# alpapad/java-rsync

Hardware: AMD Instinct MI355X
Metric: GiB/s device-resident rolling+MD5 scan (Generator block sums + Sender match scan; bytes read) (higher is better)
Workload: dtype u8

## Files before the change

### include/rsync_hip_debug.h

```cpp
#ifndef RSYNC_HIP_DEBUG_H
#define RSYNC_HIP_DEBUG_H

#include <stdint.h>

#include "rsync_hip.h"

#ifdef __cplusplus
extern "C" {
#endif

int rsh_debug_set_option(const char* name, int64_t value);
int rsh_debug_get_option(const char* name, int64_t* value);
void rsh_debug_reset_options(void);

int rsh_debug_kernel_ms(rsh_ctx* ctx, int32_t which, double* ms);

int rsh_debug_generation(rsh_ctx* ctx, int32_t set, int32_t* gen);

int rsh_debug_streams_busy(rsh_ctx* ctx, int32_t* mask);

int rsh_debug_k1_clock(rsh_ctx* ctx, const void* d_data, int64_t n, int32_t block_length, int32_t reps,
                       double* clock_ghz);

int rsh_debug_multi_selftest(const int64_t* bytes, int32_t njobs, int32_t nparts, int32_t fail_part, int32_t* part_out,
                             int32_t* order_out, int32_t* status_out);

int rsh_debug_tokens_selftest(const uint8_t* src, int64_t n, const rsh_event* ev, int64_t n_ev,
                              const uint8_t file_md5[16], int64_t from, uint8_t* out, int64_t len, int64_t span,
                              int64_t* n_desc);

int rsh_debug_sums_selftest(int32_t unframe, const rsh_header* h, int32_t* weak, uint8_t* strong, uint8_t* wire,
                            int64_t len, int64_t span, int64_t* n_desc);

typedef struct {
    int64_t pos;
    int32_t kind;
    int32_t value;
// ... 13 lines not shown
```

### java-rsync_amd/csrc/capi.cpp

```cpp
#include <hip/hip_runtime.h>
#include <immintrin.h>
#include <stdio.h>
#include <stdlib.h>
#include <string.h>

#include <algorithm>
#include <atomic>
#include <chrono>
#include <functional>
#include <thread>
#include <vector>

#include "device.h"
#include "host_md5.h"
#include "resolver.h"
#include "rsync_hip.h"

#include "ctx.h"
#include "options.h"
#include "rsync_hip_debug.h"

namespace {
int warm_calls(rsh_ctx* c) {
    const uint8_t seed[4] = {1, 2, 3, 4};
// ... 477 lines not shown
    rsh::opt_table()[i].store(value, std::memory_order_relaxed);
    return RSH_OK;
}

int rsh_debug_get_option(const char* name, int64_t* value) {
    const int i = rsh::opt_index(name);
    if (i < 0 || !value) return RSH_E_INVAL;
    *value = rsh::opt((rsh::Opt)i);
    return RSH_OK;
}

void rsh_debug_reset_options(void) {
    for (int i = 0; i < rsh::OPT_COUNT; ++i) rsh::opt_table()[i].store(rsh::opt_info()[i].def, std::memory_order_relaxed);
}

int rsh_debug_kernel_ms(rsh_ctx* ctx, int32_t which, double* ms) {
    if (!ctx || !ms || which < 0 || which > 2) return RSH_E_INVAL;
    *ms = -1.0;
    const bool timed = which == 0 ? ctx->gen_timed : which == 1 ? ctx->spec_timed : ctx->sums_timed;
    if (!timed) return RSH_OK;
    const hipEvent_t a = which == 0 ? ctx->ev_gen_a : which == 1 ? ctx->ev_k1a : ctx->ev_sums_a;
    const hipEvent_t b = which == 0 ? ctx->ev_gen_b : which == 1 ? ctx->ev_k1b : ctx->ev_sums_b;
    RSH_HIP(hipSetDevice(ctx->device));
    RSH_HIP(hipEventSynchronize(b));
    float f = 0.f;
    RSH_HIP(hipEventElapsedTime(&f, a, b));
    *ms = f;
    return RSH_OK;
}

// ... 55 lines not shown
```

### java-rsync_amd/csrc/device.h

```cpp
#pragma once
#include <hip/hip_runtime.h>
#include <stdint.h>

#include <vector>

#include "hit_cache.h"
#include "rsync_hip.h"

namespace rsh {

hipError_t launch_block_sums(const uint8_t* d_data, int64_t n, uint32_t B, uint32_t nchunks, uint32_t dl,
                             uint32_t seed_word, int32_t* d_weak, uint8_t* d_strong, hipStream_t s,
                             const int* abort_flag = nullptr, int abort_gen = 0);
void k1_timing_next(hipEvent_t start, hipEvent_t stop);
bool k1_timing_taken();

#ifdef RSH_KBENCH
hipError_t launch_block_sums_variant(int variant, const uint8_t* d_data, int64_t n, uint32_t B, uint32_t nchunks,
                                     uint32_t dl, uint32_t seed_word, int32_t* d_weak, uint8_t* d_strong,
                                     hipStream_t s, const int* abort_flag = nullptr, int abort_gen = 0);
#endif

struct K1File {
    const uint8_t* data;
// ... 41 lines not shown
struct K1Plan {
    const uint8_t* data;
    int32_t* weak;
    uint8_t* strong;
    uint32_t B, dl;
    uint32_t g0, ng;
    const int* abort = nullptr;
    int32_t file = 0;
    uint32_t nfull = 0;
};
uint32_t plan_block_sums_files(const K1File* files, int32_t nfiles, std::vector<K1Plan>* plans,
                               std::vector<K1Lane>* lanes, int* lane_align, bool* partial = nullptr);
hipError_t launch_expand_groups(const K1Plan* d_plans, uint32_t nplans, uint32_t ngroups, K1Group* d_groups,
                                hipStream_t s);
bool tail_gather_on();
hipError_t launch_block_sums_batch(const K1Group* d_groups, uint32_t ngroups, const K1Lane* d_lanes, uint32_t nlanes,
                                   int lane_align, uint32_t seed_word, hipStream_t s, const int* abort_flag = nullptr,
                                   int abort_gen = 0, bool partial = false);

hipError_t launch_chain_flags(const int32_t* d_wsrc, const uint8_t* d_ssrc, const int32_t* d_wbas,
                              const uint8_t* d_sbas, uint32_t count, uint32_t dl, uint8_t* d_flags,
                              hipStream_t s);
hipError_t launch_warm_k1(hipStream_t s);
hipError_t launch_warm_scan(hipStream_t s);
hipError_t launch_warm_chain(hipStream_t s);
hipError_t launch_warm_io(hipStream_t s);
constexpr uint32_t kStampGroups = 64, kStampLine = 16;
struct Stamp {
    uint32_t* counter;
    int* stamp;
// ... 258 lines not shown
```

### java-rsync_amd/csrc/device.hip

```cpp
#include <hip/hip_ext.h>
#include <hip/hip_runtime.h>

#include "device.h"
#include "device_common.h"
#include "md5_core.h"
#include "options.h"

#include <algorithm>
#include <type_traits>

namespace rsh {

__device__ __forceinline__ void weak_block(const uint32_t (&m)[16], int32_t& s1, int32_t& u, uint32_t off) {
    int32_t a = 0, b = 0;
#pragma unroll
    for (int j = 0; j < 16; ++j) {
        a = __builtin_amdgcn_sdot4((int)m[j], 0x01010101, a, false);
        const int w = (4 * j) | ((4 * j + 1) << 8) | ((4 * j + 2) << 16) | ((4 * j + 3) << 24);
        b = __builtin_amdgcn_sdot4((int)m[j], w, b, false);
    }
    s1 += a;
    u += (int32_t)(off * (uint32_t)a) + b;
}

// ... 193 lines not shown
    return v;
}

__device__ __forceinline__ void compiler_fence() { asm volatile("" ::: "memory"); }

__device__ __forceinline__ void md5_stream_block(Md5State& st, const uint32_t (&m)[16]) { md5_compress_rot16n(st, m); }

#ifndef RSH_K1_TAIL_PF
#define RSH_K1_TAIL_PF 2
#endif
#ifdef RSH_K1_NUMVGPR
#define K1_PIPE_ATTR __attribute__((amdgpu_num_vgpr(RSH_K1_NUMVGPR)))
#else
#define K1_PIPE_ATTR __attribute__((amdgpu_waves_per_eu(3)))
#endif
template <bool MULTI = false, bool GATHER = false, bool WEAKV = false>
__device__ __forceinline__ void block_sums_pipe_body(const uint8_t* __restrict__ data, uint32_t B, uint32_t dl,
                                                             uint32_t seed, int32_t* __restrict__ weak_out,
                                                             uint8_t* __restrict__ strong_out,
                                                             const int* abort_flag = nullptr, int abort_gen = 0,
                                                             const K1Group* __restrict__ groups = nullptr,
                                                             int64_t n = 0, uint32_t nchunks = 0,
                                                             uint32_t main_waves = 0xFFFFFFFFu,
                                                             const K1Tail* __restrict__ gt = nullptr,
                                                             uint32_t gcnt = 0, uint32_t gsel = 0xFFFFFFFFu) {
    constexpr int ROW = 9;
    constexpr int BUF = 64 * ROW;
    constexpr int TAIL_PF = RSH_K1_TAIL_PF;
    if constexpr (!MULTI && !GATHER) {
        if (blockIdx.x >= main_waves) {
            const uint32_t c = main_waves * 64u + (blockIdx.x - main_waves) * 64u + threadIdx.x;
// ... 40 lines not shown
    {
        const int m = l & 15, q = l >> 4, type = m >> 2;
#pragma unroll
        for (int w = 0; w < 4; ++w)
#pragma unroll
            for (int d = 0; d < 4; ++d) {
                uint32_t word = 0;
                if (q == (m & 3) && type == 0) word = 0x01010101u;
                else if (q == (m & 3) && type == 1)
#pragma unroll
                    for (int b = 0; b < 4; ++b) word |= (uint32_t)(16 * w + 4 * d + b) << (8 * b);
                wW[w][d] = (int)word;
            }
    }

    uint4 q[2][8];
    uint4 Wa[4];
    uint4 Wb[4];
    const __amdgpu_buffer_rsrc_t rsrc =
        __builtin_amdgcn_make_buffer_rsrc(const_cast<uint8_t*>(gdata), 0, (int)(64 * B), 0x00020000);
    const uint32_t lane_off = (uint32_t)(l >> 3) * B + 16u * (uint32_t)(l & 7);
    auto load = [&](uint4 (&dst)[8], uint32_t stg) __attribute__((always_inline)) {
#pragma unroll
        for (int j = 0; j < 8; ++j) {
            if constexpr (GATHER) {
                dst[j] = ld16<false>(rp[j] + 128u * stg);
            } else {
                const u32x4 t = __builtin_amdgcn_raw_buffer_load_b128(rsrc, lane_off + 128u * stg, (int)(j * 8u * B), 2);
                dst[j] = make_uint4(t.x, t.y, t.z, t.w);
            }
        }
    };
    auto put = [&](const uint4 (&src)[8], int buf) __attribute__((always_inline)) {
#pragma unroll
        for (int j = 0; j < 8; ++j) lds_all[buf * BUF + wr0 + j * 8 * ROW] = src[j];
    };
    auto get_words = [&](uint4 (&w)[4], int buf, int h) __attribute__((always_inline)) {
#pragma unroll
        for (int k = 0; k < 4; ++k) w[k] = lds_all[buf * BUF + rd0 + 4 * h + k];
    };
    Md5State st = md5_init();
    auto md5_block = [&](const uint4 (&w)[4]) __attribute__((always_inline)) {
        uint32_t m[16];
        unpack(w, m);
        md5_stream_block(st, m);
    };
    [[maybe_unused]] int32_t vs1 = 0, vu = 0;
    auto weak_words = [&](const uint4 (&w)[4], [[maybe_unused]] uint32_t off) __attribute__((always_inline)) {
        if constexpr (WEAKV) {
            uint32_t m[16];
            unpack(w, m);
            weak_block(m, vs1, vu, off);
        } else {
#pragma unroll
            for (int e = 0; e < 4; ++e) RW[e] += accW[e];
#pragma unroll
            for (int k = 0; k < 4; ++k) {
                const v4i32 b4 = {(int)w[k].x, (int)w[k].y, (int)w[k].z, (int)w[k].w};
                accW = __builtin_amdgcn_mfma_i32_16x16x64_i8(wW[k], b4, accW, 0, 0, 0);
            }
        }
    };
    auto stage = [&](auto pc, uint32_t si, bool has_next, bool refill) __attribute__((always_inline)) {
        constexpr int P = decltype(pc)::value;
        if (has_next) {
            put(q[P ^ 1], P ^ 1);
            if (refill) load(q[P ^ 1], si + 3);
        }
        get_words(Wb, P, 1);
        md5_block(Wa);
        weak_words(Wa, 128u * si);
        compiler_fence();
        if (has_next) get_words(Wa, P ^ 1, 0);
        md5_block(Wb);
        weak_words(Wb, 128u * si + 64u);
        compiler_fence();
// ... 11 lines not shown
    compiler_fence();
    get_words(Wa, 0, 0);
    uint32_t s = 0;
    int flag = 0;
    for (; s + 5 <= nst && flag != abort_gen; s += 2) {
        asm volatile("s_load_dword %0, %1, 0x0 glc" : "=s"(flag) : "s"(abort_flag));
        stage(std::integral_constant<int, 0>{}, s, true, true);
        stage(std::integral_constant<int, 1>{}, s + 1, true, true);
        asm volatile("s_waitcnt lgkmcnt(0)" : "+s"(flag));
    }
    if (flag == abort_gen) return;
    for (; s < nst; s += 2) {
        stage(std::integral_constant<int, 0>{}, s, s + 1 < nst, s + 3 < nst);
        if (s + 1 < nst) stage(std::integral_constant<int, 1>{}, s + 1, s + 2 < nst, s + 4 < nst);
    }
    {
        const uint64_t bits = ((uint64_t)B + 4) * 8;
        uint32_t m[16] = {seed, 0x80u, 0, 0, 0, 0, 0, 0, 0, 0, 0, 0, 0, 0, (uint32_t)bits, (uint32_t)(bits >> 32)};
        md5_compress(st, m);
    }
    int32_t s1, u;
    if constexpr (WEAKV) {
        s1 = vs1;
        u = vu;
    } else {
#pragma unroll
        for (int e = 0; e < 4; ++e) RW[e] += accW[e];
        const int n = l & 15, q = l >> 4;
        int32_t tS[4], tR[4], tW[4];
#pragma unroll
// ... 11 lines not shown
    uint32_t c = c0 + l;
    if constexpr (GATHER) {
        if ((uint32_t)l >= gcnt) return;
        if (gt) {
            const K1Tail t = gt[l];
            weak_out = t.weak;
            strong_out = t.strong;
            c = t.c;
        }
    }
    const int32_t s2 = (int32_t)(B * (uint32_t)s1 - (uint32_t)u);
    weak_out[c] = (int32_t)(((uint32_t)s1 & 0xFFFFu) | ((uint32_t)s2 << 16));
    store_digest(strong_out + (size_t)c * dl, st, dl);
}

template <bool MULTI = false>
__global__ __launch_bounds__(64) K1_PIPE_ATTR void block_sums_pipe_kernel(const uint8_t* __restrict__ data, uint32_t B, uint32_t dl,
                                                             uint32_t seed, int32_t* __restrict__ weak_out,
                                                             uint8_t* __restrict__ strong_out,
                                                             const int* abort_flag = nullptr, int abort_gen = 0,
                                                             const K1Group* __restrict__ groups = nullptr,
                                                             int64_t n = 0, uint32_t nchunks = 0,
                                                             uint32_t main_waves = 0xFFFFFFFFu) {
    block_sums_pipe_body<MULTI>(data, B, dl, seed, weak_out, strong_out, abort_flag, abort_gen, groups, n, nchunks,
                                main_waves);
}
__global__ __launch_bounds__(64) __attribute__((amdgpu_num_vgpr(256))) void block_sums_pipe_tailg_kernel(
    const uint8_t* __restrict__ data, uint32_t B, uint32_t dl, uint32_t seed, int32_t* __restrict__ weak_out,
    uint8_t* __restrict__ strong_out, const int* abort_flag, int abort_gen, int64_t n, uint32_t nchunks,
    uint32_t main_waves, uint32_t tail_full) {
    if (blockIdx.x >= main_waves) {
        const uint32_t tw = blockIdx.x - main_waves, ngw = (tail_full + 63u) / 64u;
        if (tw < ngw) {
            const uint32_t first = main_waves * 64u + 64u * tw;
            block_sums_pipe_body<false, true>(
                data + (size_t)first * B, B, dl, seed, weak_out + first, strong_out + (size_t)first * dl, abort_flag,
                abort_gen, nullptr, 0, 0, 0xFFFFFFFFu, nullptr, min(64u, tail_full - 64u * tw));
            return;
        }
        const uint32_t c = main_waves * 64u + tail_full + (tw - ngw) * 64u + threadIdx.x;
        if (c < nchunks) lane_chunk_sums<16, RSH_K1_TAIL_PF, false>(data, n, B, c, dl, seed, weak_out, strong_out);
        return;
    }
    block_sums_pipe_body<false>(data, B, dl, seed, weak_out, strong_out, abort_flag, abort_gen, nullptr, n, nchunks,
                                main_waves);
}
bool tail_gather_on() { return opt(OPT_K1_GATHER) != 0; }
#ifdef RSH_KBENCH
__global__ __launch_bounds__(64) K1_PIPE_ATTR void block_sums_pipe_weakv_kernel(
    const uint8_t* __restrict__ data, uint32_t B, uint32_t dl, uint32_t seed, int32_t* __restrict__ weak_out,
    uint8_t* __restrict__ strong_out, const int* abort_flag, int abort_gen) {
    block_sums_pipe_body<false, false, true>(data, B, dl, seed, weak_out, strong_out, abort_flag, abort_gen);
}
#endif

__global__ __launch_bounds__(64) K1_PIPE_ATTR void block_sums_pipe_clock_kernel(
    const uint8_t* __restrict__ data, uint32_t B, uint32_t dl, uint32_t seed, int32_t* __restrict__ weak_out,
    uint8_t* __restrict__ strong_out, const int* abort_flag, int abort_gen, int64_t n, uint32_t nchunks,
    unsigned long long* __restrict__ clk) {
    const uint64_t c0 = __builtin_amdgcn_s_memtime(), r0 = __builtin_amdgcn_s_memrealtime();
    block_sums_pipe_body<false>(data, B, dl, seed, weak_out, strong_out, abort_flag, abort_gen, nullptr, n, nchunks,
                                0xFFFFFFFFu);
    const uint64_t c1 = __builtin_amdgcn_s_memtime(), r1 = __builtin_amdgcn_s_memrealtime();
    if (threadIdx.x == 0) {
        atomicAdd(&clk[0], (unsigned long long)(c1 - c0));
        atomicAdd(&clk[1], (unsigned long long)(r1 - r0));
    }
}

hipError_t launch_k1_clock(const uint8_t* d_data, int64_t n, uint32_t B, uint32_t dl, uint32_t seed_word,
                           int32_t* d_weak, uint8_t* d_strong, unsigned long long* d_clk, hipStream_t s) {
    if (B == 0 || B % 128 != 0 || n <= 0 || n % (64 * (int64_t)B) != 0 || dl > 16) return hipErrorInvalidValue;
    const uint32_t nchunks = (uint32_t)(n / B), waves = nchunks / 64;
    const size_t wave_lds = 64 * 9 * sizeof(uint4);
    hipLaunchKernelGGL(block_sums_pipe_clock_kernel, dim3(waves), dim3(64), 2 * wave_lds, s, d_data, B, dl, seed_word,
                       d_weak, d_strong, never_word(), -1, n, nchunks, d_clk);
    return hipGetLastError();
}
#ifndef RSH_K1_SHIFT_VGPR
#define RSH_K1_SHIFT_VGPR 256
#endif
template <int W>
__device__ __forceinline__ void shift_wave(const uint8_t* __restrict__ gdata, uint32_t a, uint32_t B, uint32_t dl,
                                           uint32_t seed, int32_t* __restrict__ weak_out,
                                           uint8_t* __restrict__ strong_out, const int* abort_flag, int abort_gen) {
    constexpr int ROW = 17;
    extern __shared__ __attribute__((aligned(16))) uint4 lds_all[];
    const int l = threadIdx.x;
    const uint32_t nst = B >> 7;
    const uint32_t Q = a >> 4, r = a & 3;
    const int wr0 = (l >> 3) * ROW + (l & 7);
// ... 203 lines not shown
        t_k1_taken = true;
    } else {
        hipLaunchKernelGGL(kernel, grid, block, lds, s, static_cast<KArgs>(args)...);
    }
}

#ifndef RSH_KBENCH
static
#endif
hipError_t launch_block_sums_variant(int variant, const uint8_t* d_data, int64_t n, uint32_t B, uint32_t nchunks,
                                     uint32_t dl, uint32_t seed_word, int32_t* d_weak, uint8_t* d_strong,
                                     hipStream_t s, const int* abort_flag, int abort_gen) {
    if (nchunks == 0) return hipSuccess;
    const uintptr_t addr = reinterpret_cast<uintptr_t>(d_data);
    const uint32_t nst = B >> 7;
#ifdef RSH_KBENCH
    if (variant == 1010) {
        if ((B % 128) != 0 || nst < 4 || nst > 1024 || n != (int64_t)nchunks * B || nchunks % 64 != 0 || (addr % 128) != 0)
            return hipErrorInvalidValue;
        hipLaunchKernelGGL(block_sums_pipe_weakv_kernel, dim3(nchunks / 64), dim3(64), 2 * 64 * 9 * sizeof(uint4), s,
                           d_data, B, dl, seed_word, d_weak, d_strong, abort_flag ? abort_flag : never_word(),
                           abort_flag ? abort_gen : -1);
        return hipGetLastError();
    }
#endif
    const bool coalesced = variant < 0 && abort_flag && (B % 128) == 0 && nst >= 4 && nst <= 1024;
    if (coalesced && (addr % 128) != 0 && opt(OPT_K1_SHIFT) != 0) {
        hipDeviceptr_t lo = nullptr;
        size_t size = 0;
        const uint32_t a = (uint32_t)(addr % 128);
        if (hipMemGetAddressRange(&lo, &size, reinterpret_cast<hipDeviceptr_t>(const_cast<uint8_t*>(d_data))) ==
// ... 29 lines not shown
                    default:
                        k1_launch(block_sums_shift_kernel<3>, grid, dim3(64), (uint32_t)lb, s, d_data, n, a, B, nchunks,
                                  mw, dl, seed_word, d_weak, d_strong, abort_flag, abort_gen, tf);
                }
                return hipGetLastError();
            }
        }
    }
    const uint32_t waves = (uint32_t)std::min<int64_t>(n / B, nchunks) / 64;
    if (coalesced && waves > 0 && ((addr % 16) == 0 || opt(OPT_K1_UNALIGNED) != 0)) {
        const uint32_t nfullc = (uint32_t)std::min<int64_t>(n / B, nchunks);
        const size_t wave_lds = 64 * 9 * sizeof(uint4);
        const uint32_t tail_waves = (nchunks - 64 * waves + 63) / 64;
        const uint32_t tail_full = nfullc - 64 * waves, tail_short = nchunks - nfullc;
        const uint32_t gwaves = (tail_full + 63) / 64 + (tail_short + 63) / 64;
        if (tail_full > 0 && tail_gather_on() && (gwaves == tail_waves || waves + gwaves <= 2 * 4 * kCUs)) {
            k1_launch(block_sums_pipe_tailg_kernel, dim3(waves + gwaves), dim3(64), (uint32_t)(2 * wave_lds), s, d_data,
                      B, dl, seed_word, d_weak, d_strong, abort_flag, abort_gen, n, nchunks, waves, tail_full);
            return hipGetLastError();
        }
        k1_launch(block_sums_pipe_kernel<false>, dim3(waves + tail_waves), dim3(64), (uint32_t)(2 * wave_lds), s,
                  d_data, B, dl, seed_word, d_weak, d_strong, abort_flag, abort_gen, nullptr, n, nchunks, waves);
        return hipGetLastError();
    }
    const dim3 block(64);
    const dim3 grid((nchunks + 63) / 64);
    if ((B % 16) == 0 && (addr % 16) == 0) {
        hipLaunchKernelGGL((block_sums_kernel<16, 4, true>), grid, block, 0, s, d_data, n, B, nchunks, dl, seed_word,
                           d_weak, d_strong, 0u);
    } else if ((B % 4) == 0 && (addr % 4) == 0) {
        hipLaunchKernelGGL((block_sums_kernel<4, 2>), grid, block, 0, s, d_data, n, B, nchunks, dl, seed_word, d_weak,
                           d_strong, 0u);
    } else {
        hipLaunchKernelGGL((block_sums_kernel<0, 4, false>), grid, block, 0, s, d_data, n, B, nchunks, dl, seed_word,
                           d_weak, d_strong, 0u);
    }
    return hipGetLastError();
// ... 102 lines not shown
}

static const int* never_word() {
    static int* ptr[64] = {};
    int dev = 0;
    if (hipGetDevice(&dev) != hipSuccess || dev < 0 || dev >= 64) return nullptr;
    if (!ptr[dev]) {
        int* p = nullptr;
        if (hipExtMallocWithFlags(reinterpret_cast<void**>(&p), 256, hipDeviceMallocUncached) != hipSuccess) return nullptr;
        if (hipMemset(p, 0, 256) != hipSuccess) return nullptr;
        ptr[dev] = p;
    }
    return ptr[dev];
}

template <int ALIGN>
__global__ __launch_bounds__(64) __attribute__((amdgpu_num_vgpr(256))) void block_sums_pipe_multi_g_kernel(
    const K1Group* __restrict__ groups, uint32_t ngroups, const K1Lane* __restrict__ lanes, uint32_t seed,
    const int* abort_flag, int abort_gen) {
    if (blockIdx.x >= ngroups) {
        const K1Lane e = lanes[blockIdx.x - ngroups];
        const uint32_t c = e.c_first + threadIdx.x;
        if (c < e.nchunks)
            lane_chunk_sums<ALIGN == 1 ? 0 : ALIGN, ALIGN == 16 ? 4 : ALIGN == 4 ? 2 : 4, ALIGN != 1>(
                e.data, e.n, e.B, c, e.dl, seed, e.weak, e.strong);
        return;
    }
    const K1Group g = groups[blockIdx.x];
    if (g.count < 64) {
        block_sums_pipe_body<false, true>(g.data, g.B, g.dl, seed, g.weak, g.strong,
                                                           g.abort ? g.abort : abort_flag, abort_gen, nullptr, 0, 0,
                                                           0xFFFFFFFFu, nullptr, g.count);
        return;
    }
    block_sums_pipe_body<true>(nullptr, 0u, 0u, seed, nullptr, nullptr, abort_flag, abort_gen, groups);
}

hipError_t launch_block_sums_batch(const K1Group* d_groups, uint32_t ngroups, const K1Lane* d_lanes, uint32_t nlanes,
                                   int lane_align, uint32_t seed_word, hipStream_t s, const int* abort_flag,
                                   int abort_gen, bool partial) {
    const size_t lb = 2 * 64 * 9 * sizeof(uint4);
    if (!abort_flag && (abort_flag = never_word()) != nullptr) abort_gen = -1;
    if (!abort_flag) return hipErrorOutOfMemory;
    if (partial || (tail_gather_on() && nlanes > 0 && ngroups > 0)) {
        const dim3 grid(ngroups + nlanes);
        if (lane_align == 16)
            hipLaunchKernelGGL((block_sums_pipe_multi_g_kernel<16>), grid, dim3(64), lb, s, d_groups, ngroups, d_lanes,
                               seed_word, abort_flag, abort_gen);
        else if (lane_align == 4)
            hipLaunchKernelGGL((block_sums_pipe_multi_g_kernel<4>), grid, dim3(64), lb, s, d_groups, ngroups, d_lanes,
                               seed_word, abort_flag, abort_gen);
        else
            hipLaunchKernelGGL((block_sums_pipe_multi_g_kernel<1>), grid, dim3(64), lb, s, d_groups, ngroups, d_lanes,
                               seed_word, abort_flag, abort_gen);
        return hipGetLastError();
    }
    if (ngroups > 0)
        hipLaunchKernelGGL((block_sums_pipe_kernel<true>), dim3(ngroups), dim3(64), lb, s, nullptr, 0u, 0u, seed_word,
                           nullptr, nullptr, abort_flag, abort_gen, d_groups);
    if (nlanes > 0) {
        if (lane_align == 16)
            hipLaunchKernelGGL((block_sums_lane_batch_kernel<16>), dim3(nlanes), dim3(64), 0, s, d_lanes, seed_word);
        else if (lane_align == 4)
            hipLaunchKernelGGL((block_sums_lane_batch_kernel<4>), dim3(nlanes), dim3(64), 0, s, d_lanes, seed_word);
        else
            hipLaunchKernelGGL((block_sums_lane_batch_kernel<1>), dim3(nlanes), dim3(64), 0, s, d_lanes, seed_word);
    }
    return hipGetLastError();
}

hipError_t launch_block_sums(const uint8_t* d_data, int64_t n, uint32_t B, uint32_t nchunks, uint32_t dl,
                             uint32_t seed_word, int32_t* d_weak, uint8_t* d_strong, hipStream_t s,
                             const int* abort_flag, int abort_gen) {
    if (!abort_flag && (abort_flag = never_word()) != nullptr) abort_gen = -1;
// ... 32 lines not shown
```

### java-rsync_amd/csrc/options.h

```cpp
#pragma once
#include <stdint.h>
#include <string.h>

#include <atomic>

namespace rsh {

enum Opt : int {
    OPT_K1_GATHER,
    OPT_K1_SHIFT,
    OPT_K1_UNALIGNED,
    OPT_SCAN_TRACE,
    OPT_SCAN_SEGMENTED,
    OPT_SCAN_SAMPLES,
    OPT_BATCH_CHAIN,
    OPT_BATCH_CHAIN_PREFIX,
    OPT_HOST_CORES,
    OPT_FILE_TILE,
    OPT_FILE_TILE_ABOVE,
    OPT_PROBE_LONG,
    OPT_SEGMENT_BYTES,
    OPT_MD5_WIDTH,
    OPT_CHAIN_HELPERS,
    OPT_CHAIN_MAP_BYTES,
    OPT_TIME_GEN,
    OPT_BATCH_WARM,
    OPT_FAULT_INJECT,
    OPT_TOKENS_SPAN,
    OPT_TOKENS_PIECE,
    OPT_SUMS_PIECE,
    OPT_TOKENS_RUNS,
    OPT_COUNT
};

struct OptInfo {
    const char* name;
    int64_t def;
};

inline constexpr OptInfo kOpts[OPT_COUNT] = {
    {"k1_gather", 1},           {"k1_shift", 1},        {"k1_unaligned", 1},
    {"scan_trace", 0},          {"scan_segmented", 1},  {"scan_samples", 256},
    {"batch_chain", 1},         {"batch_chain_prefix", -1}, {"host_cores", 0},
    {"file_tile", 4LL << 30},   {"file_tile_above", 32LL << 30}, {"probe_long", 1},
    {"segment_bytes", 16LL << 30}, {"md5_width", 0},    {"chain_helpers", -1},
    {"chain_map_bytes", 1LL << 30}, {"time_gen", 1},    {"batch_warm", 128},
    {"fault_inject", 0},        {"tokens_span", 256LL << 10}, {"tokens_piece", 8LL << 20},
    {"sums_piece", 32LL << 20}, {"tokens_runs", 64LL << 10},
};

inline const OptInfo* opt_info() { return kOpts; }

inline std::atomic<int64_t>* opt_table() {
    static std::atomic<int64_t> v[OPT_COUNT] = {};
    static std::atomic<bool> init{false};
    if (!init.load(std::memory_order_acquire)) {
        static std::atomic_flag once = ATOMIC_FLAG_INIT;
        if (!once.test_and_set()) {
            for (int i = 0; i < OPT_COUNT; ++i) v[i].store(kOpts[i].def, std::memory_order_relaxed);
            init.store(true, std::memory_order_release);
        } else {
            while (!init.load(std::memory_order_acquire)) {
            }
// ... 15 lines not shown
```

### java-rsync_amd/rsync_hip.py

```python
import ctypes
import os
import subprocess

import numpy as np

HERE = os.path.dirname(os.path.abspath(__file__))
LIB_PATH = os.environ.get("RSH_LIB") or os.path.join(HERE, "lib", "librsynchip.so")

RSH_OK, RSH_E_INVAL, RSH_E_PROTOCOL, RSH_E_OVERFLOW, RSH_E_NOSPACE, RSH_E_DEVICE, RSH_E_NOMEM, RSH_E_BUSY = \
    0, -1, -2, -3, -4, -5, -6, -7
RSH_E_NOTFOUND, RSH_E_OPEN, RSH_E_NOSOURCE = -8, -9, -10
EV_LITERAL, EV_MATCH = 1, 2


class ProtocolError(Exception):
    """RsyncProtocolException (Connection.receiveChecksumHeader, Connection.java:28-38)."""


class FileViewNotFound(FileNotFoundError):
    """RSH_E_NOTFOUND (io/FileViewNotFound: new FileView on a missing file, FileView.java:74-75)."""


class FileViewOpenFailed(OSError):
    """RSH_E_OPEN (io/FileViewOpenFailed, FileView.java:76-78)."""
# ... 120 lines not shown
                        ("count", "<i4"), ("reserved", "<i4")])

EXPORTS = ["rsh_abi_version", "rsh_strerror", "rsh_last_error", "rsh_device_count", "rsh_ctx_create", "rsh_ctx_destroy",
           "rsh_ctx_stream", "rsh_block_length_for", "rsh_digest_length_for", "rsh_header_make",
           "rsh_header_validate", "rsh_block_sums", "rsh_block_sums_device", "rsh_ctx_sync", "rsh_ctx_trim", "rsh_match_scan",
           "rsh_match_scan_device", "rsh_match_scan_tiled", "rsh_fetch_events", "rsh_file_md5", "rsh_tokens_size", "rsh_tokens_write", "rsh_generator_bytes",
           "rsh_block_sums_batch_device", "rsh_match_scan_batch_device", "rsh_receiver_combine",
           "rsh_receiver_combine_device", "rsh_receiver_combine_batch", "rsh_block_sums_file", "rsh_match_scan_file", "rsh_block_sums_pieces", "rsh_match_scan_pieces", "rsh_block_sums_batch", "rsh_match_scan_batch", "rsh_block_sums_batch_multi", "rsh_match_scan_batch_multi", "rsh_receiver_combine_batch_multi", "rsh_shard_files", "rsh_file_md5_batch", "rsh_dev_alloc", "rsh_dev_free", "rsh_memcpy_h2d", "rsh_memcpy_d2h", "rsh_fill_splitmix_device",
           "rsh_tokens_write_device", "rsh_tokens_write_kept", "rsh_tokens_write_batch_device",
           "rsh_sums_wire_size", "rsh_header_from_wire", "rsh_sums_frame_device", "rsh_sums_unframe_device",
           "rsh_block_sums_batch_wire", "rsh_match_scan_batch_wire", "rsh_block_sums_batch_wire_multi",
           "rsh_match_scan_batch_wire_multi", "rsh_tokens_frame_device", "rsh_receiver_combine_resident"]
DEBUG_EXPORTS = ["rsh_debug_set_option", "rsh_debug_get_option", "rsh_debug_reset_options", "rsh_debug_k1_clock",
                 "rsh_debug_streams_busy", "rsh_debug_kernel_ms", "rsh_debug_multi_selftest", "rsh_debug_generation",
                 "rsh_debug_tokens_selftest", "rsh_debug_sums_selftest", "rsh_debug_tokens_scan_selftest",
                 "rsh_debug_untokens_selftest"]

_LIB = None


def build(force=False):
    cmd = ["make", "-s", "-C", HERE] + (["-B"] if force else [])
    subprocess.run(cmd, check=True)


def stale_sources():
    import hashlib
    stamp = os.path.splitext(LIB_PATH)[0] + ".srchash"
    if not os.path.exists(stamp):
        return []
    out = []
# ... 62 lines not shown
        "rsh_match_scan_batch": ([P, ctypes.POINTER(ScanBatchJob), I32, P, ctypes.POINTER(ScanStats)], ctypes.c_int),
        "rsh_block_sums_batch_multi": ([ctypes.POINTER(P), I32, ctypes.POINTER(BlockBatchJob), I32, P], ctypes.c_int),
        "rsh_match_scan_batch_multi": ([ctypes.POINTER(P), I32, ctypes.POINTER(ScanBatchJob), I32, P,
                                        ctypes.POINTER(ScanStats)], ctypes.c_int),
        "rsh_receiver_combine_batch_multi": ([ctypes.POINTER(P), I32, ctypes.POINTER(CombineJob), I32], ctypes.c_int),
        "rsh_shard_files": ([P, I32, I32, P], ctypes.c_int),
        "rsh_file_md5_batch": ([ctypes.POINTER(Md5Job), I32, I32], ctypes.c_int),
        "rsh_dev_alloc": ([P, I64, ctypes.POINTER(P)], ctypes.c_int),
        "rsh_dev_free": ([P, P], ctypes.c_int),
        "rsh_memcpy_h2d": ([P, P, P, I64], ctypes.c_int),
        "rsh_memcpy_d2h": ([P, P, P, I64], ctypes.c_int),
        "rsh_fill_splitmix_device": ([P, P, I64, ctypes.c_uint64, I64], ctypes.c_int),
        "rsh_debug_set_option": ([ctypes.c_char_p, I64], ctypes.c_int),
        "rsh_debug_get_option": ([ctypes.c_char_p, ctypes.POINTER(I64)], ctypes.c_int),
        "rsh_debug_reset_options": ([], None),
        "rsh_debug_k1_clock": ([P, P, I64, I32, I32, ctypes.POINTER(ctypes.c_double)], ctypes.c_int),
        "rsh_debug_streams_busy": ([P, ctypes.POINTER(ctypes.c_int32)], ctypes.c_int),
        "rsh_debug_generation": ([P, I32, ctypes.POINTER(ctypes.c_int32)], ctypes.c_int),
        "rsh_debug_kernel_ms": ([P, I32, ctypes.POINTER(ctypes.c_double)], ctypes.c_int),
        "rsh_debug_multi_selftest": ([P, I32, I32, I32, P, P, P], ctypes.c_int),
        "rsh_tokens_write_device": ([P, P, I64, P, I64, P, I64, P, I64], ctypes.c_int),
        "rsh_tokens_write_kept": ([P, P, I64, P, I64, P, I64], ctypes.c_int),
        "rsh_tokens_write_batch_device": ([P, ctypes.POINTER(TokenJob), I32], ctypes.c_int),
        "rsh_debug_tokens_selftest": ([P, I64, P, I64, P, I64, P, I64, I64, ctypes.POINTER(I64)], ctypes.c_int),
        "rsh_sums_wire_size": ([HP], I64),
        "rsh_header_from_wire": ([P, HP], ctypes.c_int),
        "rsh_sums_frame_device": ([P, HP, P, P, P, I64], ctypes.c_int),
        "rsh_sums_unframe_device": ([P, HP, P, I64, P, P], ctypes.c_int),
        "rsh_block_sums_batch_wire": ([P, ctypes.POINTER(BlockWireJob), I32, P], ctypes.c_int),
        "rsh_match_scan_batch_wire": ([P, ctypes.POINTER(SendJob), I32, P, ctypes.POINTER(ScanStats)], ctypes.c_int),
# ... 714 lines not shown
```

Baseline: 5142.

## Stream K1 block-sum input via buffer_load-to-LDS DMA with swizzled staging

Adds a DMA path to the block-sums pipeline kernel. Raw buffer_load ... lds instructions copy each 128-byte stage straight into LDS using an XOR-swizzled layout, instead of routing the data through VGPRs and then writing it to LDS. Reads are double-buffered with vmcnt-based waits and abort polling through scalar loads. The goal is to cut VGPR traffic and instruction overhead in the memory-bound MD5/weak-sum loop. The cost is hand-written inline asm that manipulates m0, a fixed 16 KiB LDS footprint, and a new option, enabled by default, that falls back to the old register path.

```diff
diff --git a/include/rsync_hip_debug.h b/include/rsync_hip_debug.h
--- a/include/rsync_hip_debug.h
+++ b/include/rsync_hip_debug.h
@@ -21,6 +21,8 @@
 
 int rsh_debug_k1_clock(rsh_ctx* ctx, const void* d_data, int64_t n, int32_t block_length, int32_t reps,
                        double* clock_ghz);
+
+int32_t rsh_debug_k1_dma_swizzle(int32_t what, int32_t chunk, int32_t index);
 
 int rsh_debug_multi_selftest(const int64_t* bytes, int32_t njobs, int32_t nparts, int32_t fail_part, int32_t* part_out,
                              int32_t* order_out, int32_t* status_out);
diff --git a/java-rsync_amd/csrc/capi.cpp b/java-rsync_amd/csrc/capi.cpp
--- a/java-rsync_amd/csrc/capi.cpp
+++ b/java-rsync_amd/csrc/capi.cpp
@@ -515,6 +515,12 @@
     for (int i = 0; i < rsh::OPT_COUNT; ++i) rsh::opt_table()[i].store(rsh::opt_info()[i].def, std::memory_order_relaxed);
 }
 
+int32_t rsh_debug_k1_dma_swizzle(int32_t what, int32_t chunk, int32_t index) {
+    if (what < 0 || what > 2 || chunk < 0 || chunk > 63 || index < 0 || index > 7) return -1;
+    const uint32_t c = (uint32_t)chunk, i = (uint32_t)index;
+    return (int32_t)(what == 0 ? rsh::k1_dma_piece(c, i) : what == 1 ? rsh::k1_dma_slot(c, i) : rsh::k1_dma_lds_byte(c, i));
+}
+
 int rsh_debug_kernel_ms(rsh_ctx* ctx, int32_t which, double* ms) {
     if (!ctx || !ms || which < 0 || which > 2) return RSH_E_INVAL;
     *ms = -1.0;
diff --git a/java-rsync_amd/csrc/device.h b/java-rsync_amd/csrc/device.h
--- a/java-rsync_amd/csrc/device.h
+++ b/java-rsync_amd/csrc/device.h
@@ -79,6 +79,11 @@
 hipError_t launch_expand_groups(const K1Plan* d_plans, uint32_t nplans, uint32_t ngroups, K1Group* d_groups,
                                 hipStream_t s);
 bool tail_gather_on();
+constexpr uint32_t K1_DMA_STAGE = 8192;
+constexpr uint32_t k1_dma_piece(uint32_t c, uint32_t p) { return p ^ ((c >> 1) & 7u); }
+constexpr uint32_t k1_dma_slot(uint32_t c, uint32_t k) { return k ^ ((c >> 1) & 7u); }
+constexpr uint32_t k1_dma_lds_byte(uint32_t c, uint32_t slot) { return 128u * c + 16u * slot; }
+bool k1_dma_on();
 hipError_t launch_block_sums_batch(const K1Group* d_groups, uint32_t ngroups, const K1Lane* d_lanes, uint32_t nlanes,
                                    int lane_align, uint32_t seed_word, hipStream_t s, const int* abort_flag = nullptr,
                                    int abort_gen = 0, bool partial = false);
diff --git a/java-rsync_amd/csrc/device.hip b/java-rsync_amd/csrc/device.hip
--- a/java-rsync_amd/csrc/device.hip
+++ b/java-rsync_amd/csrc/device.hip
@@ -231,7 +231,7 @@
 #else
 #define K1_PIPE_ATTR __attribute__((amdgpu_waves_per_eu(3)))
 #endif
-template <bool MULTI = false, bool GATHER = false, bool WEAKV = false>
+template <bool MULTI = false, bool GATHER = false, bool WEAKV = false, bool DMA = false, int DIAG = 0>
 __device__ __forceinline__ void block_sums_pipe_body(const uint8_t* __restrict__ data, uint32_t B, uint32_t dl,
                                                              uint32_t seed, int32_t* __restrict__ weak_out,
                                                              uint8_t* __restrict__ strong_out,
@@ -302,8 +302,140 @@
             }
     }
 
+    Md5State st = md5_init();
+    auto md5_block = [&](const uint4 (&w)[4]) __attribute__((always_inline)) {
+        if constexpr (DIAG == 2) {
+#pragma unroll
+            for (int k = 0; k < 4; ++k) st.a ^= w[k].x ^ w[k].y ^ w[k].z ^ w[k].w;
+            return;
+        }
+        uint32_t m[16];
+        unpack(w, m);
+        md5_stream_block(st, m);
+    };
+    [[maybe_unused]] int32_t vs1 = 0, vu = 0;
+    auto weak_words = [&](const uint4 (&w)[4], [[maybe_unused]] uint32_t off) __attribute__((always_inline)) {
+        if constexpr (DIAG == 2) return;
+        if constexpr (WEAKV) {
+            uint32_t m[16];
+            unpack(w, m);
+            weak_block(m, vs1, vu, off);
+        } else {
+#pragma unroll
+            for (int e = 0; e < 4; ++e) RW[e] += accW[e];
+#pragma unroll
+            for (int k = 0; k < 4; ++k) {
+                const v4i32 b4 = {(int)w[k].x, (int)w[k].y, (int)w[k].z, (int)w[k].w};
+                accW = __builtin_amdgcn_mfma_i32_16x16x64_i8(wW[k], b4, accW, 0, 0, 0);
+            }
+        }
+    };
+    uint4 Wa[4];
+    if constexpr (DMA) {
+        static_assert(!GATHER && !WEAKV, "the DMA form is the main waves' form only");
+        B = (uint32_t)__builtin_amdgcn_readfirstlane((int)B);
+        const uint64_t ga = reinterpret_cast<uint64_t>(gdata);
+        const v4i32 desc = {__builtin_amdgcn_readfirstlane((int)(uint32_t)ga),
+                            __builtin_amdgcn_readfirstlane((int)((uint32_t)(ga >> 32) & 0xFFFFu)),
+                            DIAG == 1 ? 0 : (int)(64u * B),
+                            0x00020000};
+        const uint32_t lds0 = __builtin_amdgcn_readfirstlane(
+            (int)(uint32_t)reinterpret_cast<uintptr_t>((__attribute__((address_space(3))) void*)lds_all));
+        const uint32_t voff = (uint32_t)(l >> 3) * B + 16u * k1_dma_piece((uint32_t)(l >> 3), (uint32_t)(l & 7));
+        const uint32_t so1 = 8u * B, so2 = 16u * B, so3 = 24u * B, so4 = 32u * B, so5 = 40u * B, so6 = 48u * B,
+                       so7 = 56u * B;
+        auto dma = [&](int slot, uint32_t stg) __attribute__((always_inline)) {
+            uint32_t keep;
+            const uint32_t ve = voff + 128u * stg, vo = ve ^ 64u;
+            asm volatile(
+                "s_nop 4\n\t"
+                "s_waitcnt lgkmcnt(0)\n\t"
+                "s_mov_b32 %0, m0\n\t"
+                "s_mov_b32 m0, %4\n\t"
+                "s_nop 0\n\t"
+                "buffer_load_dwordx4 %2, %1, 0 offen nt lds\n\t"
+                "s_add_u32 m0, m0, 0x400\n\t"
+                "s_nop 0\n\t"
+                "buffer_load_dwordx4 %3, %1, %5 offen nt lds\n\t"
+                "s_add_u32 m0, m0, 0x400\n\t"
+                "s_nop 0\n\t"
+                "buffer_load_dwordx4 %2, %1, %6 offen nt lds\n\t"
+                "s_add_u32 m0, m0, 0x400\n\t"
+                "s_nop 0\n\t"
+                "buffer_load_dwordx4 %3, %1, %7 offen nt lds\n\t"
+                "s_add_u32 m0, m0, 0x400\n\t"
+                "s_nop 0\n\t"
+                "buffer_load_dwordx4 %2, %1, %8 offen nt lds\n\t"
+                "s_add_u32 m0, m0, 0x400\n\t"
+                "s_nop 0\n\t"
+                "buffer_load_dwordx4 %3, %1, %9 offen nt lds\n\t"
+                "s_add_u32 m0, m0, 0x400\n\t"
+                "s_nop 0\n\t"
+                "buffer_load_dwordx4 %2, %1, %10 offen nt lds\n\t"
+                "s_add_u32 m0, m0, 0x400\n\t"
+                "s_nop 0\n\t"
+                "buffer_load_dwordx4 %3, %1, %11 offen nt lds\n\t"
+                "s_mov_b32 m0, %0"
+                : "=&s"(keep)
+                : "s"(desc), "v"(ve), "v"(vo), "s"(lds0 + (uint32_t)slot * K1_DMA_STAGE), "s"(so1), "s"(so2), "s"(so3),
+                  "s"(so4), "s"(so5), "s"(so6), "s"(so7)
+                : "memory", "scc");
+        };
+        const uint32_t rdx = ((uint32_t)l >> 1) & 7u;
+        auto get_stage = [&](uint4 (&w0)[4], uint4 (&w1)[4], int slot) __attribute__((always_inline)) {
+#pragma unroll
+            for (int k = 0; k < 4; ++k) w0[k] = lds_all[slot * 512 + 8 * l + (int)((uint32_t)k ^ rdx)];
+#pragma unroll
+            for (int k = 0; k < 4; ++k) w1[k] = lds_all[slot * 512 + 8 * l + (int)((uint32_t)(4 + k) ^ rdx)];
+        };
+        uint4 Wb[2][4];
+        int flag = 0;
+        auto stage = [&](auto pc, uint32_t si, bool has_next, bool refill, bool poll) __attribute__((always_inline)) {
+            constexpr int P = decltype(pc)::value;
+            if (refill) dma(P, si + 2);
+            if (poll) asm volatile("s_load_dword %0, %1, 0x0 glc" : "=s"(flag) : "s"(abort_flag));
+            md5_block(Wa);
+            weak_words(Wa, 128u * si);
+            compiler_fence();
+            if (has_next) {
+                if (refill) asm volatile("s_waitcnt vmcnt(8)" : "+v"(st.a) : : "memory");
+                else asm volatile("s_waitcnt vmcnt(0)" : "+v"(st.a) : : "memory");
+                get_stage(Wa, Wb[P ^ 1], P ^ 1);
+                __builtin_amdgcn_sched_barrier(0);
+            }
+            md5_block(Wb[P]);
+            weak_words(Wb[P], 128u * si + 64u);
+            compiler_fence();
+        };
+        dma(0, 0);
+        dma(1, 1);
+        if constexpr (MULTI) {
+            int f0;
+            asm volatile("s_load_dword %0, %1, 0x0 glc\n\ts_waitcnt lgkmcnt(0)" : "=s"(f0) : "s"(abort_flag));
+            if (f0 == abort_gen) {
+                asm volatile("s_waitcnt vmcnt(0)" ::: "memory");
+                return;
+            }
+        }
+        asm volatile("s_waitcnt vmcnt(8)" ::: "memory");
+        get_stage(Wa, Wb[0], 0);
+        uint32_t s = 0;
+        for (; s + 5 <= nst && flag != abort_gen; s += 2) {
+            stage(std::integral_constant<int, 0>{}, s, true, true, true);
+            stage(std::integral_constant<int, 1>{}, s + 1, true, true, false);
+            asm volatile("s_waitcnt lgkmcnt(0)" : "+s"(flag));
+        }
+        if (flag == abort_gen) {
+            asm volatile("s_waitcnt vmcnt(0)" ::: "memory");
+            return;
+        }
+        for (; s < nst; s += 2) {
+            stage(std::integral_constant<int, 0>{}, s, s + 1 < nst, s + 2 < nst, false);
+            if (s + 1 < nst) stage(std::integral_constant<int, 1>{}, s + 1, s + 2 < nst, s + 3 < nst, false);
+        }
+        asm volatile("s_waitcnt vmcnt(0)" ::: "memory");
+    } else {
     uint4 q[2][8];
-    uint4 Wa[4];
     uint4 Wb[4];
     const __amdgpu_buffer_rsrc_t rsrc =
         __builtin_amdgcn_make_buffer_rsrc(const_cast<uint8_t*>(gdata), 0, (int)(64 * B), 0x00020000);
@@ -326,28 +458,6 @@
     auto get_words = [&](uint4 (&w)[4], int buf, int h) __attribute__((always_inline)) {
 #pragma unroll
         for (int k = 0; k < 4; ++k) w[k] = lds_all[buf * BUF + rd0 + 4 * h + k];
-    };
-    Md5State st = md5_init();
-    auto md5_block = [&](const uint4 (&w)[4]) __attribute__((always_inline)) {
-        uint32_t m[16];
-        unpack(w, m);
-        md5_stream_block(st, m);
-    };
-    [[maybe_unused]] int32_t vs1 = 0, vu = 0;
-    auto weak_words = [&](const uint4 (&w)[4], [[maybe_unused]] uint32_t off) __attribute__((always_inline)) {
-        if constexpr (WEAKV) {
-            uint32_t m[16];
-            unpack(w, m);
-            weak_block(m, vs1, vu, off);
-        } else {
-#pragma unroll
-            for (int e = 0; e < 4; ++e) RW[e] += accW[e];
-#pragma unroll
-            for (int k = 0; k < 4; ++k) {
-                const v4i32 b4 = {(int)w[k].x, (int)w[k].y, (int)w[k].z, (int)w[k].w};
-                accW = __builtin_amdgcn_mfma_i32_16x16x64_i8(wW[k], b4, accW, 0, 0, 0);
-            }
-        }
     };
     auto stage = [&](auto pc, uint32_t si, bool has_next, bool refill) __attribute__((always_inline)) {
         constexpr int P = decltype(pc)::value;
@@ -389,6 +499,7 @@
         stage(std::integral_constant<int, 0>{}, s, s + 1 < nst, s + 3 < nst);
         if (s + 1 < nst) stage(std::integral_constant<int, 1>{}, s + 1, s + 2 < nst, s + 4 < nst);
     }
+    }
     {
         const uint64_t bits = ((uint64_t)B + 4) * 8;
         uint32_t m[16] = {seed, 0x80u, 0, 0, 0, 0, 0, 0, 0, 0, 0, 0, 0, 0, (uint32_t)bits, (uint32_t)(bits >> 32)};
@@ -430,6 +541,22 @@
     store_digest(strong_out + (size_t)c * dl, st, dl);
 }
 
+constexpr bool k1_dma_swizzle_ok() {
+    for (uint32_t k = 0; k < 8; ++k)
+        for (uint32_t g = 0; g < 4; ++g) {
+            uint32_t spans = 0;
+            for (uint32_t i = 0; i < 16; ++i) {
+                const uint32_t c = 16 * g + i, slot = k1_dma_slot(c, k);
+                if (slot > 7 || k1_dma_piece(c, slot) != k) return false;
+                spans |= 1u << ((k1_dma_lds_byte(c, slot) >> 4) & 15u);
+            }
+            if (spans != 0xFFFFu) return false;
+        }
+    return true;
+}
+static_assert(k1_dma_swizzle_ok(), "K1 DMA image: bank conflict or slot / piece mismatch");
+bool k1_dma_on() { return opt(OPT_K1_DMA) != 0; }
+
 template <bool MULTI = false>
 __global__ __launch_bounds__(64) K1_PIPE_ATTR void block_sums_pipe_kernel(const uint8_t* __restrict__ data, uint32_t B, uint32_t dl,
                                                              uint32_t seed, int32_t* __restrict__ weak_out,
@@ -438,10 +565,20 @@
                                                              const K1Group* __restrict__ groups = nullptr,
                                                              int64_t n = 0, uint32_t nchunks = 0,
                                                              uint32_t main_waves = 0xFFFFFFFFu) {
+    block_sums_pipe_body<MULTI, false, false, true>(data, B, dl, seed, weak_out, strong_out, abort_flag, abort_gen,
+                                                    groups, n, nchunks, main_waves);
+}
+template <bool MULTI = false>
+__global__ __launch_bounds__(64) K1_PIPE_ATTR void block_sums_pipe_reg_kernel(
+    const uint8_t* __restrict__ data, uint32_t B, uint32_t dl, uint32_t seed, int32_t* __restrict__ weak_out,
+    uint8_t* __restrict__ strong_out, const int* abort_flag = nullptr, int abort_gen = 0,
+    const K1Group* __restrict__ groups = nullptr, int64_t n = 0, uint32_t nchunks = 0,
+    uint32_t main_waves = 0xFFFFFFFFu) {
     block_sums_pipe_body<MULTI>(data, B, dl, seed, weak_out, strong_out, abort_flag, abort_gen, groups, n, nchunks,
                                 main_waves);
 }
-__global__ __launch_bounds__(64) __attribute__((amdgpu_num_vgpr(256))) void block_sums_pipe_tailg_kernel(
+template <bool DMA>
+__device__ __forceinline__ void block_sums_pipe_tailg_body(
     const uint8_t* __restrict__ data, uint32_t B, uint32_t dl, uint32_t seed, int32_t* __restrict__ weak_out,
     uint8_t* __restrict__ strong_out, const int* abort_flag, int abort_gen, int64_t n, uint32_t nchunks,
     uint32_t main_waves, uint32_t tail_full) {
@@ -458,8 +595,22 @@
         if (c < nchunks) lane_chunk_sums<16, RSH_K1_TAIL_PF, false>(data, n, B, c, dl, seed, weak_out, strong_out);
         return;
     }
-    block_sums_pipe_body<false>(data, B, dl, seed, weak_out, strong_out, abort_flag, abort_gen, nullptr, n, nchunks,
-                                main_waves);
+    block_sums_pipe_body<false, false, false, DMA>(data, B, dl, seed, weak_out, strong_out, abort_flag, abort_gen,
+                                                   nullptr, n, nchunks, main_waves);
+}
+__global__ __launch_bounds__(64) __attribute__((amdgpu_num_vgpr(256))) void block_sums_pipe_tailg_kernel(
+    const uint8_t* __restrict__ data, uint32_t B, uint32_t dl, uint32_t seed, int32_t* __restrict__ weak_out,
+    uint8_t* __restrict__ strong_out, const int* abort_flag, int abort_gen, int64_t n, uint32_t nchunks,
+    uint32_t main_waves, uint32_t tail_full) {
+    block_sums_pipe_tailg_body<true>(data, B, dl, seed, weak_out, strong_out, abort_flag, abort_gen, n, nchunks,
+                                     main_waves, tail_full);
+}
+__global__ __launch_bounds__(64) __attribute__((amdgpu_num_vgpr(256))) void block_sums_pipe_tailg_reg_kernel(
+    const uint8_t* __restrict__ data, uint32_t B, uint32_t dl, uint32_t seed, int32_t* __restrict__ weak_out,
+    uint8_t* __restrict__ strong_out, const int* abort_flag, int abort_gen, int64_t n, uint32_t nchunks,
+    uint32_t main_waves, uint32_t tail_full) {
+    block_sums_pipe_tailg_body<false>(data, B, dl, seed, weak_out, strong_out, abort_flag, abort_gen, n, nchunks,
+                                      main_waves, tail_full);
 }
 bool tail_gather_on() { return opt(OPT_K1_GATHER) != 0; }
 #ifdef RSH_KBENCH
@@ -468,15 +619,23 @@
     uint8_t* __restrict__ strong_out, const int* abort_flag, int abort_gen) {
     block_sums_pipe_body<false, false, true>(data, B, dl, seed, weak_out, strong_out, abort_flag, abort_gen);
 }
+template <int DIAG>
+__global__ __launch_bounds__(64) K1_PIPE_ATTR void block_sums_pipe_diag_kernel(
+    const uint8_t* __restrict__ data, uint32_t B, uint32_t dl, uint32_t seed, int32_t* __restrict__ weak_out,
+    uint8_t* __restrict__ strong_out, const int* abort_flag, int abort_gen) {
+    block_sums_pipe_body<false, false, false, true, DIAG>(data, B, dl, seed, weak_out, strong_out, abort_flag,
+                                                          abort_gen);
+}
 #endif
 
+template <bool DMA>
 __global__ __launch_bounds__(64) K1_PIPE_ATTR void block_sums_pipe_clock_kernel(
     const uint8_t* __restrict__ data, uint32_t B, uint32_t dl, uint32_t seed, int32_t* __restrict__ weak_out,
     uint8_t* __restrict__ strong_out, const int* abort_flag, int abort_gen, int64_t n, uint32_t nchunks,
     unsigned long long* __restrict__ clk) {
     const uint64_t c0 = __builtin_amdgcn_s_memtime(), r0 = __builtin_amdgcn_s_memrealtime();
-    block_sums_pipe_body<false>(data, B, dl, seed, weak_out, strong_out, abort_flag, abort_gen, nullptr, n, nchunks,
-                                0xFFFFFFFFu);
+    block_sums_pipe_body<false, false, false, DMA>(data, B, dl, seed, weak_out, strong_out, abort_flag, abort_gen,
+                                                   nullptr, n, nchunks, 0xFFFFFFFFu);
     const uint64_t c1 = __builtin_amdgcn_s_memtime(), r1 = __builtin_amdgcn_s_memrealtime();
     if (threadIdx.x == 0) {
         atomicAdd(&clk[0], (unsigned long long)(c1 - c0));
@@ -488,9 +647,12 @@
                            int32_t* d_weak, uint8_t* d_strong, unsigned long long* d_clk, hipStream_t s) {
     if (B == 0 || B % 128 != 0 || n <= 0 || n % (64 * (int64_t)B) != 0 || dl > 16) return hipErrorInvalidValue;
     const uint32_t nchunks = (uint32_t)(n / B), waves = nchunks / 64;
-    const size_t wave_lds = 64 * 9 * sizeof(uint4);
-    hipLaunchKernelGGL(block_sums_pipe_clock_kernel, dim3(waves), dim3(64), 2 * wave_lds, s, d_data, B, dl, seed_word,
-                       d_weak, d_strong, never_word(), -1, n, nchunks, d_clk);
+    if (k1_dma_on() && reinterpret_cast<uintptr_t>(d_data) % 16 == 0)
+        hipLaunchKernelGGL(block_sums_pipe_clock_kernel<true>, dim3(waves), dim3(64), 2 * K1_DMA_STAGE, s, d_data, B, dl,
+                           seed_word, d_weak, d_strong, never_word(), -1, n, nchunks, d_clk);
+    else
+        hipLaunchKernelGGL(block_sums_pipe_clock_kernel<false>, dim3(waves), dim3(64), 2 * 64 * 9 * sizeof(uint4), s,
+                           d_data, B, dl, seed_word, d_weak, d_strong, never_word(), -1, n, nchunks, d_clk);
     return hipGetLastError();
 }
 #ifndef RSH_K1_SHIFT_VGPR
@@ -724,7 +886,24 @@
     if (nchunks == 0) return hipSuccess;
     const uintptr_t addr = reinterpret_cast<uintptr_t>(d_data);
     const uint32_t nst = B >> 7;
+    bool dma_on = k1_dma_on();
 #ifdef RSH_KBENCH
+    if (variant == 1020 || variant == 1021) {
+        dma_on = variant == 1020;
+        variant = -1;
+    }
+    if (variant == 1023 || variant == 1024) {
+        if ((B % 128) != 0 || nst < 4 || nst > 1024 || n != (int64_t)nchunks * B || nchunks % 64 != 0 || (addr % 16) != 0)
+            return hipErrorInvalidValue;
+        const int* word = abort_flag ? abort_flag : never_word();
+        if (variant == 1023)
+            hipLaunchKernelGGL(block_sums_pipe_diag_kernel<1>, dim3(nchunks / 64), dim3(64), 2 * K1_DMA_STAGE, s, d_data, B,
+                               dl, seed_word, d_weak, d_strong, word, abort_flag ? abort_gen : -1);
+        else
+            hipLaunchKernelGGL(block_sums_pipe_diag_kernel<2>, dim3(nchunks / 64), dim3(64), 2 * K1_DMA_STAGE, s, d_data, B,
+                               dl, seed_word, d_weak, d_strong, word, abort_flag ? abort_gen : -1);
+        return hipGetLastError();
+    }
     if (variant == 1010) {
         if ((B % 128) != 0 || nst < 4 || nst > 1024 || n != (int64_t)nchunks * B || nchunks % 64 != 0 || (addr % 128) != 0)
             return hipErrorInvalidValue;
@@ -784,13 +963,19 @@
         const uint32_t tail_waves = (nchunks - 64 * waves + 63) / 64;
         const uint32_t tail_full = nfullc - 64 * waves, tail_short = nchunks - nfullc;
         const uint32_t gwaves = (tail_full + 63) / 64 + (tail_short + 63) / 64;
+        const bool dma = dma_on && (addr % 16) == 0;
         if (tail_full > 0 && tail_gather_on() && (gwaves == tail_waves || waves + gwaves <= 2 * 4 * kCUs)) {
-            k1_launch(block_sums_pipe_tailg_kernel, dim3(waves + gwaves), dim3(64), (uint32_t)(2 * wave_lds), s, d_data,
-                      B, dl, seed_word, d_weak, d_strong, abort_flag, abort_gen, n, nchunks, waves, tail_full);
+            k1_launch(dma ? block_sums_pipe_tailg_kernel : block_sums_pipe_tailg_reg_kernel, dim3(waves + gwaves),
+                      dim3(64), (uint32_t)(2 * wave_lds), s, d_data, B, dl, seed_word, d_weak, d_strong, abort_flag,
+                      abort_gen, n, nchunks, waves, tail_full);
             return hipGetLastError();
         }
-        k1_launch(block_sums_pipe_kernel<false>, dim3(waves + tail_waves), dim3(64), (uint32_t)(2 * wave_lds), s,
-                  d_data, B, dl, seed_word, d_weak, d_strong, abort_flag, abort_gen, nullptr, n, nchunks, waves);
+        if (dma)
+            k1_launch(block_sums_pipe_kernel<false>, dim3(waves + tail_waves), dim3(64), 2 * K1_DMA_STAGE, s, d_data, B,
+                      dl, seed_word, d_weak, d_strong, abort_flag, abort_gen, nullptr, n, nchunks, waves);
+        else
+            k1_launch(block_sums_pipe_reg_kernel<false>, dim3(waves + tail_waves), dim3(64), (uint32_t)(2 * wave_lds), s,
+                      d_data, B, dl, seed_word, d_weak, d_strong, abort_flag, abort_gen, nullptr, n, nchunks, waves);
         return hipGetLastError();
     }
     const dim3 block(64);
@@ -923,7 +1108,7 @@
     return ptr[dev];
 }
 
-template <int ALIGN>
+template <int ALIGN, bool DMA = true>
 __global__ __launch_bounds__(64) __attribute__((amdgpu_num_vgpr(256))) void block_sums_pipe_multi_g_kernel(
     const K1Group* __restrict__ groups, uint32_t ngroups, const K1Lane* __restrict__ lanes, uint32_t seed,
     const int* abort_flag, int abort_gen) {
@@ -942,31 +1127,49 @@
                                                            0xFFFFFFFFu, nullptr, g.count);
         return;
     }
-    block_sums_pipe_body<true>(nullptr, 0u, 0u, seed, nullptr, nullptr, abort_flag, abort_gen, groups);
+    block_sums_pipe_body<true, false, false, DMA>(nullptr, 0u, 0u, seed, nullptr, nullptr, abort_flag, abort_gen, groups);
 }
 
 hipError_t launch_block_sums_batch(const K1Group* d_groups, uint32_t ngroups, const K1Lane* d_lanes, uint32_t nlanes,
                                    int lane_align, uint32_t seed_word, hipStream_t s, const int* abort_flag,
                                    int abort_gen, bool partial) {
     const size_t lb = 2 * 64 * 9 * sizeof(uint4);
+    const bool dma = k1_dma_on();
     if (!abort_flag && (abort_flag = never_word()) != nullptr) abort_gen = -1;
     if (!abort_flag) return hipErrorOutOfMemory;
     if (partial || (tail_gather_on() && nlanes > 0 && ngroups > 0)) {
         const dim3 grid(ngroups + nlanes);
-        if (lane_align == 16)
-            hipLaunchKernelGGL((block_sums_pipe_multi_g_kernel<16>), grid, dim3(64), lb, s, d_groups, ngroups, d_lanes,
-                               seed_word, abort_flag, abort_gen);
-        else if (lane_align == 4)
-            hipLaunchKernelGGL((block_sums_pipe_multi_g_kernel<4>), grid, dim3(64), lb, s, d_groups, ngroups, d_lanes,
-                               seed_word, abort_flag, abort_gen);
+        if (dma) {
+            if (lane_align == 16)
+                hipLaunchKernelGGL((block_sums_pipe_multi_g_kernel<16>), grid, dim3(64), lb, s, d_groups, ngroups,
+                                   d_lanes, seed_word, abort_flag, abort_gen);
+            else if (lane_align == 4)
+                hipLaunchKernelGGL((block_sums_pipe_multi_g_kernel<4>), grid, dim3(64), lb, s, d_groups, ngroups, d_lanes,
+                                   seed_word, abort_flag, abort_gen);
+            else
+                hipLaunchKernelGGL((block_sums_pipe_multi_g_kernel<1>), grid, dim3(64), lb, s, d_groups, ngroups, d_lanes,
+                                   seed_word, abort_flag, abort_gen);
+        } else {
+            if (lane_align == 16)
+                hipLaunchKernelGGL((block_sums_pipe_multi_g_kernel<16, false>), grid, dim3(64), lb, s, d_groups, ngroups,
+                                   d_lanes, seed_word, abort_flag, abort_gen);
+            else if (lane_align == 4)
+                hipLaunchKernelGGL((block_sums_pipe_multi_g_kernel<4, false>), grid, dim3(64), lb, s, d_groups, ngroups,
+                                   d_lanes, seed_word, abort_flag, abort_gen);
+            else
+                hipLaunchKernelGGL((block_sums_pipe_multi_g_kernel<1, false>), grid, dim3(64), lb, s, d_groups, ngroups,
+                                   d_lanes, seed_word, abort_flag, abort_gen);
+        }
+        return hipGetLastError();
+    }
+    if (ngroups > 0) {
+        if (dma)
+            hipLaunchKernelGGL((block_sums_pipe_kernel<true>), dim3(ngroups), dim3(64), 2 * K1_DMA_STAGE, s, nullptr, 0u,
+                               0u, seed_word, nullptr, nullptr, abort_flag, abort_gen, d_groups);
         else
-            hipLaunchKernelGGL((block_sums_pipe_multi_g_kernel<1>), grid, dim3(64), lb, s, d_groups, ngroups, d_lanes,
-                               seed_word, abort_flag, abort_gen);
-        return hipGetLastError();
-    }
-    if (ngroups > 0)
-        hipLaunchKernelGGL((block_sums_pipe_kernel<true>), dim3(ngroups), dim3(64), lb, s, nullptr, 0u, 0u, seed_word,
-                           nullptr, nullptr, abort_flag, abort_gen, d_groups);
+            hipLaunchKernelGGL((block_sums_pipe_reg_kernel<true>), dim3(ngroups), dim3(64), lb, s, nullptr, 0u, 0u,
+                               seed_word, nullptr, nullptr, abort_flag, abort_gen, d_groups);
+    }
     if (nlanes > 0) {
         if (lane_align == 16)
             hipLaunchKernelGGL((block_sums_lane_batch_kernel<16>), dim3(nlanes), dim3(64), 0, s, d_lanes, seed_word);
diff --git a/java-rsync_amd/csrc/options.h b/java-rsync_amd/csrc/options.h
--- a/java-rsync_amd/csrc/options.h
+++ b/java-rsync_amd/csrc/options.h
@@ -30,6 +30,7 @@
     OPT_TOKENS_PIECE,
     OPT_SUMS_PIECE,
     OPT_TOKENS_RUNS,
+    OPT_K1_DMA,
     OPT_COUNT
 };
 
@@ -46,7 +47,7 @@
     {"segment_bytes", 16LL << 30}, {"md5_width", 0},    {"chain_helpers", -1},
     {"chain_map_bytes", 1LL << 30}, {"time_gen", 1},    {"batch_warm", 128},
     {"fault_inject", 0},        {"tokens_span", 256LL << 10}, {"tokens_piece", 8LL << 20},
-    {"sums_piece", 32LL << 20}, {"tokens_runs", 64LL << 10},
+    {"sums_piece", 32LL << 20}, {"tokens_runs", 64LL << 10}, {"k1_dma", 1},
 };
 
 inline const OptInfo* opt_info() { return kOpts; }
diff --git a/java-rsync_amd/rsync_hip.py b/java-rsync_amd/rsync_hip.py
--- a/java-rsync_amd/rsync_hip.py
+++ b/java-rsync_amd/rsync_hip.py
@@ -158,7 +158,7 @@
 DEBUG_EXPORTS = ["rsh_debug_set_option", "rsh_debug_get_option", "rsh_debug_reset_options", "rsh_debug_k1_clock",
                  "rsh_debug_streams_busy", "rsh_debug_kernel_ms", "rsh_debug_multi_selftest", "rsh_debug_generation",
                  "rsh_debug_tokens_selftest", "rsh_debug_sums_selftest", "rsh_debug_tokens_scan_selftest",
-                 "rsh_debug_untokens_selftest"]
+                 "rsh_debug_untokens_selftest", "rsh_debug_k1_dma_swizzle"]
 
 _LIB = None
 
@@ -251,6 +251,7 @@
         "rsh_debug_set_option": ([ctypes.c_char_p, I64], ctypes.c_int),
         "rsh_debug_get_option": ([ctypes.c_char_p, ctypes.POINTER(I64)], ctypes.c_int),
         "rsh_debug_reset_options": ([], None),
+        "rsh_debug_k1_dma_swizzle": ([I32, I32, I32], ctypes.c_int32),
         "rsh_debug_k1_clock": ([P, P, I64, I32, I32, ctypes.POINTER(ctypes.c_double)], ctypes.c_int),
         "rsh_debug_streams_busy": ([P, ctypes.POINTER(ctypes.c_int32)], ctypes.c_int),
         "rsh_debug_generation": ([P, I32, ctypes.POINTER(ctypes.c_int32)], ctypes.c_int),
```

New measurement: 5284 (median of 6 runs). 2.8% higher.
